# tashoyan/locations-recommender

Hardware: AMD Instinct MI355X
Metric: KNN person-pair cosines/s (cosine place+category, combine, top-K) (higher is better)
Workload: dtype u16 dot (exact, packed) / f64 cosine

## Files before the change

### include/locrec.h

```cpp
#ifndef LOCREC_H
#define LOCREC_H

#include <stdint.h>

#ifdef __cplusplus
extern "C" {
#endif

#define LOCREC_OK 0
#define LOCREC_E_INVALID_ARG 1
#define LOCREC_E_NOT_FOUND 2
#define LOCREC_E_DEVICE 3
#define LOCREC_E_OOM 4
#define LOCREC_E_ARITHMETIC 5

#define LOCREC_MEM_HOST 0
#define LOCREC_MEM_DEVICE 1

const char *locrec_last_error(void);
const char *locrec_version(void);

int32_t locrec_device_count(int32_t *out_count);
int32_t locrec_set_device(int32_t ordinal);
int32_t locrec_device_allocations(int64_t *out_count);
// ... 29 lines not shown

int32_t locrec_knn_destroy(locrec_knn_index *index);

int32_t locrec_knn_info(const locrec_knn_index *index, int64_t *out_n,
                        int64_t *out_scan_bytes, int32_t *out_packed);

int32_t locrec_knn_batch_scan_bytes(const locrec_knn_index *index, int64_t *out_scan_bytes);

int32_t locrec_knn_ht_image_info(const locrec_knn_index *index, int64_t *out_head_words, int64_t *out_tail_postings,
                                 int64_t *out_wide_rows);

int32_t locrec_knn_ht_multiplied_words(const locrec_knn_index *index, int64_t *out_words);

int32_t locrec_knn_ht_slice_counts(const locrec_knn_index *index, int64_t capacity, int32_t *out_place, int32_t *out_category,
                                   int64_t *out_slices);

int32_t locrec_knn_ht_last_hits(locrec_knn_index *index, int64_t nq, int64_t tile_capacity, int64_t off_capacity,
                                int64_t hit_capacity, int32_t *out_query_tile, int64_t *out_tiles, int32_t *out_slice0,
                                int32_t *out_nslices, int64_t *out_tile_base, uint32_t *out_off, uint32_t *out_hits,
                                int64_t *out_total);

int32_t locrec_knn_scan_plan(const locrec_knn_index *index, int32_t *out_kernel, int32_t *out_mode,
                             int32_t *out_query_tile, int32_t *out_waves_per_block);

int32_t locrec_knn_vector_lengths(locrec_knn_index *index, double *out_place_lengths,
                                  double *out_category_lengths);

int32_t locrec_knn_cosine_similarity(locrec_knn_index *index, int64_t person_a, int64_t person_b,
                                     double *out_place_cosine, double *out_category_cosine);

// ... 369 lines not shown
```

### locations-recommender_amd/_lib.py

```python
import ctypes as C
import os

import numpy as np

_HERE = os.path.dirname(os.path.abspath(__file__))
LIB_PATH = os.environ.get("LOCREC_LIB_PATH") or os.path.join(_HERE, "liblocrec.so")

OK, E_INVALID_ARG, E_NOT_FOUND, E_DEVICE, E_OOM, E_ARITHMETIC = 0, 1, 2, 3, 4, 5
MEM_HOST, MEM_DEVICE = 0, 1
KNN_BATCH_MAX_K = 1024
RANK_BATCH_MAX_N = 256


class IllegalArgumentException(ValueError):
    """What the reference throws for a failed require() or an unknown id
    (KnnRecommender.scala:17-20,83; StochasticRecommender.scala:33-34,70)."""


class LocrecRuntimeError(RuntimeError):
    """Device / allocation failures (the JNI shim maps these to RuntimeException)."""


_i64p = C.POINTER(C.c_int64)
_i32p = C.POINTER(C.c_int32)
# ... 13 lines not shown
    "locrec_cache_clear": [],
    "locrec_cache_stats": [_i64p, _i64p, _i64p, _i64p, _i64p],
    "locrec_knn_create": [C.c_int64, _i64p, _i64p, _i32p, _f64p, C.c_int32, _i64p, _i32p, _f64p, C.c_int32,
                          _i64p, _i64p, _i64p, C.POINTER(C.c_void_p)],
    "locrec_knn_create_from_device": [C.c_int64, C.c_void_p, C.c_void_p, C.c_void_p, C.c_void_p, C.c_int32, C.c_void_p, C.c_void_p,
                                      C.c_void_p, C.c_int32, C.c_void_p, C.c_void_p, C.c_void_p, C.POINTER(C.c_void_p)],
    "locrec_knn_destroy": [C.c_void_p],
    "locrec_knn_info": [C.c_void_p, _i64p, _i64p, _i32p],
    "locrec_knn_vector_lengths": [C.c_void_p, _f64p, _f64p],
    "locrec_knn_cosine_similarity": [C.c_void_p, C.c_int64, C.c_int64, _f64p, _f64p],
    "locrec_knn_scan_plan": [C.c_void_p, _i32p, _i32p, _i32p, _i32p],
    "locrec_knn_batch_scan_bytes": [C.c_void_p, _i64p],
    "locrec_knn_ht_image_info": [C.c_void_p, _i64p, _i64p, _i64p],
    "locrec_knn_ht_multiplied_words": [C.c_void_p, _i64p],
    "locrec_knn_ht_slice_counts": [C.c_void_p, C.c_int64, _i32p, _i32p, _i64p],
    "locrec_knn_ht_last_hits": [C.c_void_p, C.c_int64, C.c_int64, C.c_int64, C.c_int64, _i32p, _i64p, _i32p, _i32p, _i64p,
                                C.POINTER(C.c_uint32), C.POINTER(C.c_uint32), _i64p],
    "locrec_knn_query": [C.c_void_p, C.c_int64, C.c_double, C.c_double, C.c_int64, _i64p, _f64p, _i64p],
    "locrec_knn_recommend": [C.c_void_p, C.c_int64, C.c_double, C.c_double, C.c_int64, _i64p, _f64p, _i64p],
    "locrec_knn_recommend_batch": [C.c_void_p, C.c_int64, _i64p, C.c_double, C.c_double, C.c_int64,
                                   _i64p, _i64p, _f64p, _i64p],
    "locrec_knn_recommend_range_async": [C.c_void_p, C.c_int64, C.c_int64, C.c_double, C.c_double, C.c_int64],
    "locrec_knn_fetch_recommend": [C.c_void_p, C.c_int64, _i64p, _i64p, _f64p, _i64p],
    "locrec_knn_recommend_ranked_batch": [C.c_void_p, C.c_int64, _i64p, C.c_double, C.c_double, C.c_int64,
                                          C.c_int64, _i64p, _i64p, _i64p, C.c_int64, _i64p, _f64p, _i64p],
    "locrec_knn_fetch_ranked": [C.c_void_p, C.c_int64, C.c_int64, _i64p, _i64p, _i64p, C.c_int64, _i64p, _f64p, _i64p],
    "locrec_knn_recommend_ranked_batch_unvisited": [C.c_void_p, C.c_int64, _i64p, C.c_double, C.c_double, C.c_int64,
                                                    C.c_int64, _i64p, _i64p, _i64p, C.c_int64, _i64p, _f64p, _i64p],
    "locrec_knn_fetch_ranked_unvisited": [C.c_void_p, C.c_int64, C.c_int64, _i64p, _i64p, _i64p, C.c_int64, _i64p, _f64p, _i64p],
    "locrec_knn_query_shard": [C.c_void_p, C.c_int64, C.c_double, C.c_double, C.c_int64, C.c_int32, C.c_int32,
# ... 210 lines not shown
```

### locations-recommender_amd/csrc/knn.hip

```cpp

#include <algorithm>
#include <chrono>
#include <cstring>
#include <cmath>
#include <cstdlib>
#include <memory>
#include <new>
#include <numeric>
#include <type_traits>
#include <unordered_map>

#include "knn_index.h"

namespace {

using namespace locrec;

constexpr uint32_t kEmpty = 0xFFFFFFFFu;
constexpr int kMergeCap = 8192;
constexpr int kAggCap = 4096;
constexpr int kDirectMaxBytes = cfg::kDirectMaxBytes;
constexpr int kLdsSoftLimit = 64 * 1024;
constexpr int kLdsHardLimit = 160 * 1024;

struct Family {
    const uint32_t *sell;
// ... 1296 lines not shown
    ix->no_direct8 = std::getenv("LOCREC_KNN_NO_DIRECT8") != nullptr;
    ix->no_pack = std::getenv("LOCREC_KNN_NO_PACK") != nullptr;
    ix->no_seed = std::getenv("LOCREC_KNN_NO_SEED") != nullptr;
    ix->ht_round4 = std::getenv("LOCREC_KNN_HT_ROUND4") != nullptr;
    ix->no_tile_special = std::getenv("LOCREC_KNN_NO_TILE_SPECIAL") != nullptr;
    if (const char *e = std::getenv("LOCREC_KNN_SEED_MIN_SLICES")) ix->seed_min_slices = std::max(1, std::atoi(e));
    if (const char *e = std::getenv("LOCREC_KNN_SEED_SAMPLE")) ix->seed_sample_slices = std::max(8, std::atoi(e));
    ix->force_dense_query = std::getenv("LOCREC_KNN_FORCE_DENSE_QUERY") != nullptr;
    ix->ht.v1 = std::getenv("LOCREC_KNN_HT_V1") != nullptr;
    if (const char *e = std::getenv("LOCREC_KNN_HT_W")) {
        const int w = std::atoi(e);
        if (w == 6 || w == 8 || w == 12) ix->ht.waves = w;
    }
    if (ix->ht.v1) ix->ht.waves = 8;
    ix->ht.pre_v1 = std::getenv("LOCREC_KNN_HT_PRE_V1") != nullptr;
    if (const char *e = std::getenv("LOCREC_KNN_HT_PRE_STAGE"))
        ix->ht.pre_stage = std::min(kHtPreStageMax, std::max(kHtPreStageMin, std::atoi(e)));
    ix->force_generic = std::getenv("LOCREC_KNN_FORCE_GENERIC") != nullptr;
    ix->no_pack16 = std::getenv("LOCREC_KNN_NO_PACK16") != nullptr;
    ix->no_pop = std::getenv("LOCREC_KNN_NO_POP") != nullptr;
    ix->no_row_fallback = std::getenv("LOCREC_KNN_NO_ROW_FALLBACK") != nullptr;
    if (const char *e = std::getenv("LOCREC_KNN_HT_H")) ix->env_ht_h = std::max(4, std::atoi(e));
    if (const char *e = std::getenv("LOCREC_KNN_POP_H")) ix->env_pop_h = std::max(64, std::atoi(e));
    if (const char *e = std::getenv("LOCREC_KNN_BLOCKS")) ix->env_blocks = std::max(1, std::atoi(e));
    if (const char *e = std::getenv("LOCREC_KNN_FLUSH")) {
        const int v = std::atoi(e);
        if (v >= 1 && v <= 64 && (v & (v - 1)) == 0) ix->env_flush = v;
    }
    if (const char *e = std::getenv("LOCREC_KNN_ENTER")) ix->env_enter = std::max(0, std::atoi(e));
}
// ... 111 lines not shown
extern "C" int32_t locrec_knn_ht_slice_counts(const locrec_knn_index *ix, int64_t capacity, int32_t *out_place, int32_t *out_category,
                                              int64_t *out_slices) try
{
    if (!ix || !out_slices || capacity < 0 || (capacity > 0 && (!out_place || !out_category)))
        return fail(LOCREC_E_INVALID_ARG, "NULL argument");
    const bool have = ix->ht.ready && !ix->no_ht;
    const int64_t ns = have ? (int64_t)ix->ht.slice_cnt.size() : 0;
    *out_slices = ns;
    for (int64_t sl = 0; sl < std::min(ns, capacity); ++sl) {
        out_place[sl] = (int32_t)(ix->ht.slice_cnt[(size_t)sl] & 0xFFFFu);
        out_category[sl] = (int32_t)(ix->ht.slice_cnt[(size_t)sl] >> 16);
    }
    return LOCREC_OK;
} LOCREC_CATCH_ALL

extern "C" int32_t locrec_knn_scan_plan(const locrec_knn_index *ix, int32_t *out_kernel, int32_t *out_mode,
                                        int32_t *out_query_tile, int32_t *out_waves_per_block) try
{
    if (!ix) return fail(LOCREC_E_INVALID_ARG, "index is NULL");
    if (out_kernel) *out_kernel = ix->last_plan_kernel;
    if (out_mode) *out_mode = ix->last_plan_mode;
    if (out_query_tile) *out_query_tile = ix->last_plan_qt;
    if (out_waves_per_block) *out_waves_per_block = ix->last_plan_waves;
    return LOCREC_OK;
} LOCREC_CATCH_ALL

extern "C" int32_t locrec_knn_vector_lengths(locrec_knn_index *ix, double *out_p, double *out_c) try
{
    if (!ix) return fail(LOCREC_E_INVALID_ARG, "index is NULL");
    LOCREC_HIP_TRY(hipSetDevice(ix->device));
// ... 260 lines not shown
    std::vector<int64_t> ids((size_t)keff);
    std::vector<double> sims((size_t)keff);
    int64_t cnt = 0;
    LOCREC_TRY(locrec_knn_fetch_topk(ix, 1, keff, ids.data(), sims.data(), &cnt));
    const int64_t cap = *inout_count;
    for (int64_t i = 0; i < std::min(cap, cnt); ++i) {
        if (out_ids) out_ids[i] = ids[i];
        if (out_sims) out_sims[i] = sims[i];
    }
    *inout_count = cnt;
    return LOCREC_OK;
} LOCREC_CATCH_ALL

namespace {

int32_t enqueue_aggregate(locrec_knn_index *ix, int64_t nq, int K)
{
    hipStream_t s = ix->stream;
    const int64_t tmax = std::min<int64_t>((int64_t)K * std::max<int64_t>(1, ix->max_r_nnz), kAggCap);
    const int M = pow2ceil((int)std::max<int64_t>(2, tmax));
    LOCREC_TRY(ix->agg_place.reserve((size_t)nq * M));
    LOCREC_TRY(ix->agg_est.reserve((size_t)nq * M));
    LOCREC_TRY(ix->agg_n.reserve((size_t)nq));
    LOCREC_TRY(ix->agg_overflow.reserve((size_t)nq));
    const int M1 = std::min(M, 2048);
    const int threads1 = (M1 < M && K <= 512) ? 512 : kAggThreads;
    const int64_t nplaces = (int64_t)ix->cplace_ids.size();
    auto key32 = [&](int cap) { return ceil_log2i(nplaces + 2) + ceil_log2i(cap) <= 32; };
    auto lds_of = [&](int cap) { return (size_t)cap * (key32(cap) ? 14 : 18) + 8 + (size_t)K * 16 + (size_t)(K + 1) * 4 + 16; };
    const size_t lds_full = lds_of(M);
    auto launch = [&](int cap, int threads, int redo) -> int32_t {
        const size_t lds = lds_of(cap);
        if (key32(cap)) {
            if (lds > 64 * 1024)
                LOCREC_HIP_TRY(hipFuncSetAttribute(reinterpret_cast<const void *>(knn_aggregate<uint32_t>),
                                                   hipFuncAttributeMaxDynamicSharedMemorySize, (int)lds));
            hipLaunchKernelGGL(knn_aggregate<uint32_t>, dim3((unsigned)nq), dim3(threads), lds, s, ix->out_rows.p, ix->out_sims.p,
                               ix->out_cnt.p, K, ix->r_ptr.p, ix->r_pidx.p, ix->r_rating.p, ix->cplace_dev.p, cap,
                               ix->agg_place.p, ix->agg_est.p, ix->agg_n.p, ix->agg_overflow.p, (int64_t)M, redo, ceil_log2i(cap));
        } else {
            if (lds > 64 * 1024)
                LOCREC_HIP_TRY(hipFuncSetAttribute(reinterpret_cast<const void *>(knn_aggregate<uint64_t>),
                                                   hipFuncAttributeMaxDynamicSharedMemorySize, (int)lds));
            hipLaunchKernelGGL(knn_aggregate<uint64_t>, dim3((unsigned)nq), dim3(threads), lds, s, ix->out_rows.p, ix->out_sims.p,
                               ix->out_cnt.p, K, ix->r_ptr.p, ix->r_pidx.p, ix->r_rating.p, ix->cplace_dev.p, cap,
                               ix->agg_place.p, ix->agg_est.p, ix->agg_n.p, ix->agg_overflow.p, (int64_t)M, redo, 16);
        }
        return LOCREC_OK;
    };
    (void)lds_full;
    LOCREC_TRY(launch(M1, threads1, 0));
    if (M1 < M) LOCREC_TRY(launch(M, kAggThreads, 1));
    LOCREC_HIP_TRY(hipGetLastError());
    ix->agg_M = M;
    ix->have_agg = true;
    return LOCREC_OK;
}

int32_t enqueue_large_k_batch(locrec_knn_index *ix, const std::vector<int32_t> &rows, double pw, double cw, int64_t k)
{
    const int64_t nq = (int64_t)rows.size();
    ix->agg_rows = rows;
    ix->agg_first = -1;
    ix->agg_pw = pw;
    ix->agg_cw = cw;
    ix->last_nq = nq;
    ix->last_k = k;
    ix->single_pending = false;
// ... 282 lines not shown
            return fail(LOCREC_E_INVALID_ARG, "neighbour %lld is listed twice", (long long)ix->ids_row[*dup]);
    }
    LOCREC_HIP_TRY(hipSetDevice(ix->device));
    hipStream_t s = ix->stream;
    ix->have_result = false;
    ix->single_pending = false;
    if (n_neighbours <= LOCREC_KNN_BATCH_MAX_K) {
        const int K = (int)n_neighbours;
        const int64_t cnt = n_neighbours;
        LOCREC_TRY(ix->out_rows.reserve((size_t)K));
        LOCREC_TRY(ix->out_sims.reserve((size_t)K));
        LOCREC_TRY(ix->out_cnt.reserve(1));
        LOCREC_HIP_TRY(hipMemcpyAsync(ix->out_rows.p, rows.data(), (size_t)K * 4, hipMemcpyHostToDevice, s));
        LOCREC_HIP_TRY(hipMemcpyAsync(ix->out_sims.p, similarities, (size_t)K * 8, hipMemcpyHostToDevice, s));
        LOCREC_HIP_TRY(hipMemcpyAsync(ix->out_cnt.p, &cnt, 8, hipMemcpyHostToDevice, s));
        const int64_t tmax = std::min<int64_t>((int64_t)K * std::max<int64_t>(1, ix->max_r_nnz), kAggCap);
        const int M = pow2ceil((int)std::max<int64_t>(2, tmax));
        LOCREC_TRY(ix->agg_place.reserve((size_t)M));
        LOCREC_TRY(ix->agg_est.reserve((size_t)M));
        LOCREC_TRY(ix->agg_n.reserve(1));
        LOCREC_TRY(ix->agg_overflow.reserve(1));
        const size_t lds = (size_t)M * 18 + 8 + (size_t)K * 16 + (size_t)(K + 1) * 4 + 16;
        if (lds > 64 * 1024)
            LOCREC_HIP_TRY(hipFuncSetAttribute(reinterpret_cast<const void *>(knn_aggregate<uint64_t>),
                                               hipFuncAttributeMaxDynamicSharedMemorySize, (int)lds));
        hipLaunchKernelGGL(knn_aggregate<uint64_t>, dim3(1), dim3(kAggThreads), lds, s, ix->out_rows.p, ix->out_sims.p,
                           ix->out_cnt.p, K, ix->r_ptr.p, ix->r_pidx.p, ix->r_rating.p, ix->cplace_dev.p, M,
                           ix->agg_place.p, ix->agg_est.p, ix->agg_n.p, ix->agg_overflow.p, (int64_t)M, 0, 16);
        LOCREC_HIP_TRY(hipGetLastError());
        int64_t nout = 0;
        int32_t overflow = 0;
        std::vector<int64_t> hp((size_t)M);
        std::vector<double> he((size_t)M);
        LOCREC_HIP_TRY(hipMemcpyAsync(&nout, ix->agg_n.p, 8, hipMemcpyDeviceToHost, s));
        LOCREC_HIP_TRY(hipMemcpyAsync(&overflow, ix->agg_overflow.p, 4, hipMemcpyDeviceToHost, s));
        LOCREC_HIP_TRY(hipMemcpyAsync(hp.data(), ix->agg_place.p, (size_t)M * 8, hipMemcpyDeviceToHost, s));
        LOCREC_HIP_TRY(hipMemcpyAsync(he.data(), ix->agg_est.p, (size_t)M * 8, hipMemcpyDeviceToHost, s));
        LOCREC_HIP_TRY(hipStreamSynchronize(s));
        if (!overflow) {
            const int64_t w = std::min(*inout_count, nout);
            if (w > 0 && out_places) std::copy(hp.begin(), hp.begin() + w, out_places);
            if (w > 0 && out_ratings) std::copy(he.begin(), he.begin() + w, out_ratings);
            *inout_count = nout;
            return LOCREC_OK;
// ... 11 lines not shown
    if (!ix) return fail(LOCREC_E_INVALID_ARG, "index is NULL");
    if (!inout_count) return fail(LOCREC_E_INVALID_ARG, "inout_count is NULL");
    LOCREC_TRY(check_params(pw, cw, k));
    int32_t row = 0;
    LOCREC_TRY(find_query_row(ix, person_id, &row));
    const int64_t keff = std::min<int64_t>(k, std::max<int64_t>(1, ix->n - 1));
    LOCREC_HIP_TRY(hipSetDevice(ix->device));
    if (keff > LOCREC_KNN_BATCH_MAX_K)
        return knn_large_recommend(ix, row, pw, cw, keff, out_places, out_ratings, inout_count);
    hipStream_t s = ix->stream;
    static const bool dbg_timing = debug_env("LOCREC_DEBUG_TIMING") != nullptr;
    const auto tp0 = std::chrono::steady_clock::now();
    LOCREC_TRY(enqueue_topk(ix, nullptr, row, 1, ix->fp.nnz[row], ix->fc.nnz[row], pw, cw, keff));
    const auto tp1 = std::chrono::steady_clock::now();
    const int K = (int)keff;
    const int64_t tmax = std::min<int64_t>((int64_t)K * std::max<int64_t>(1, ix->max_r_nnz), kAggCap);
    const int M = pow2ceil((int)std::max<int64_t>(2, tmax));
    LOCREC_TRY(ix->agg_place.reserve((size_t)M));
    LOCREC_TRY(ix->agg_est.reserve((size_t)M));
    LOCREC_TRY(ix->agg_n.reserve(1));
    LOCREC_TRY(ix->agg_overflow.reserve(1));
    const size_t lds = (size_t)M * 18 + 8 + (size_t)K * 16 + (size_t)(K + 1) * 4 + 16;
    if (lds > 64 * 1024)
        LOCREC_HIP_TRY(hipFuncSetAttribute(reinterpret_cast<const void *>(knn_aggregate<uint64_t>),
                                           hipFuncAttributeMaxDynamicSharedMemorySize, (int)lds));
    unsigned char *agg_host = nullptr;
    if (ix->single_pending && !ix->last_scan_fast && (size_t)M * 16 + 64 <= locrec_knn_index::kStageBytes && stage_of(ix) &&
        ix->h_stage_dev && !ix->no_pack)
        agg_host = ix->h_stage_dev;
    hipLaunchKernelGGL(knn_aggregate<uint64_t>, dim3(1), dim3(kAggThreads), lds, s, ix->out_rows.p, ix->out_sims.p,
                       ix->out_cnt.p, K, ix->r_ptr.p, ix->r_pidx.p, ix->r_rating.p, ix->cplace_dev.p, M,
                       ix->agg_place.p, ix->agg_est.p, ix->agg_n.p, ix->agg_overflow.p, (int64_t)M, 0, 16, agg_host,
                       ix->sel1.p + 4, M);
    LOCREC_HIP_TRY(hipGetLastError());
    const auto tp2 = std::chrono::steady_clock::now();
    int64_t nout = 0;
    int32_t overflow = 0, overflow1 = 0, qoverflow = 0;
    std::vector<int64_t> hp_v;
    std::vector<double> he_v;
    const int64_t *hp = nullptr;
    const double *he = nullptr;
    unsigned char *st = (size_t)M * 16 + 64 <= locrec_knn_index::kStageBytes ? stage_of(ix) : nullptr;
    int64_t *p_nout = &nout;
    int32_t *p_flags = nullptr;
    int32_t local_flags[3] = {0, 0, 0};
    if (st) {
        p_nout = reinterpret_cast<int64_t *>(st);
        p_flags = reinterpret_cast<int32_t *>(st + 16);
        hp = reinterpret_cast<const int64_t *>(st + 64);
// ... 69 lines not shown
```

### locations-recommender_amd/csrc/knn_aggregate.h

```cpp
#pragma once

__device__ __forceinline__ int block_exclusive_scan(int v, int *wtot, int *total)
{
    const int lane = threadIdx.x & 63, wave = threadIdx.x >> 6, nw = blockDim.x >> 6;
    int inc = v;
#pragma unroll
    for (int d = 1; d < 64; d <<= 1) {
        const int o = __shfl_up(inc, d);
        if (lane >= d) inc += o;
    }
    if (lane == 63) wtot[wave] = inc;
    __syncthreads();
    if (threadIdx.x == 0) {
        int acc = 0;
        for (int w = 0; w < nw; ++w) {
            const int t = wtot[w];
            wtot[w] = acc;
            acc += t;
        }
        wtot[16] = acc;
    }
    __syncthreads();
    *total = wtot[16];
    return wtot[wave] + inc - v;
}

constexpr int kAggThreads = 1024;

template <typename KeyT>
__global__ __launch_bounds__(kAggThreads) void knn_aggregate(
    const int32_t *nb_rows, const double *nb_sims, const int64_t *nb_cnt, int32_t K,
    const int64_t *r_ptr, const int32_t *r_pidx, const double *r_rating, const int64_t *cplace_ids,
    int32_t M , int64_t *out_place, double *out_est, int64_t *out_n,
    int32_t *out_overflow, int64_t out_stride, int32_t redo_only, int32_t fbits,
    unsigned char *host = nullptr , const int32_t *host_flag_src = nullptr, int32_t host_cap = 0)
{
    if (redo_only && out_overflow[blockIdx.x] == 0) return;
    if (host && threadIdx.x == 0 && host_flag_src) *reinterpret_cast<int32_t *>(host + 20) = *host_flag_src;
    extern __shared__ __align__(16) unsigned char smem[];
    KeyT *key = reinterpret_cast<KeyT *>(smem);
    double *wrv = reinterpret_cast<double *>(smem + (((size_t)M * sizeof(KeyT) + 7) & ~(size_t)7));
    unsigned short *av = reinterpret_cast<unsigned short *>(wrv + M);
    int64_t *rbase = reinterpret_cast<int64_t *>(reinterpret_cast<unsigned char *>(av) + (((size_t)M * 2 + 7) & ~(size_t)7));
    double *simv = reinterpret_cast<double *>(rbase + K);
    int32_t *off = reinterpret_cast<int32_t *>(simv + K);
    const int q = blockIdx.x;
    const int tid = threadIdx.x;
    const int m = max(0, (int)nb_cnt[q]);
    const int32_t *rows = nb_rows + (int64_t)q * K;
    const double *sims = nb_sims + (int64_t)q * K;
// ... 7 lines not shown
    }
    int Tsum = 0;
    const int myoff = block_exclusive_scan(mycnt, wtot, &Tsum);
    if (tid < m) off[tid] = myoff;
    if (tid == 0) off[m] = Tsum;
    __syncthreads();
    const int T = min(Tsum, M + 1);
    if (T > M) {
        if (tid == 0) {
            out_overflow[q] = 1;
            out_n[q] = 0;
            if (host) {
                *reinterpret_cast<int32_t *>(host + 16) = 1;
                *reinterpret_cast<int64_t *>(host) = 0;
            }
        }
        return;
    }
    int n2 = 2;
    while (n2 < T) n2 <<= 1;
    auto neighbour_of = [&](int f) {
        int a = 0, b = m;
        while (b - a > 1) {
            const int mid = (a + b) >> 1;
            if (off[mid] <= f) a = mid; else b = mid;
        }
        return a;
    };
    for (int f = tid; f < n2; f += blockDim.x) {
        KeyT k = ~(KeyT)0;
        if (f < T) {
            const int a = neighbour_of(f);
            const int64_t e = rbase[a] + (f - off[a]);
// ... 68 lines not shown
                ss = ss + simv[av[f]];
            }
            const int64_t place = cplace_ids[pk];
            const double est = ws / ss;
            out_place[(int64_t)q * out_stride + o] = place;
            out_est[(int64_t)q * out_stride + o] = est;
            if (host) {
                h_place[o] = place;
                h_est[o] = est;
            }
            ++o;
        }
    }
}

__global__ __launch_bounds__(256) void knn_agg_compact(const int64_t *place, const double *est, const int64_t *out_n,
                                                       const int64_t *off, int64_t stride, int64_t *dense_place,
                                                       double *dense_est)
{
    const int q = blockIdx.x;
    const int64_t n = out_n[q], o = off[q];
    for (int64_t i = threadIdx.x; i < n; i += blockDim.x) {
        dense_place[o + i] = place[(int64_t)q * stride + i];
        dense_est[o + i] = est[(int64_t)q * stride + i];
    }
}

__global__ void knn_mark_absent(const double *norm_p, const double *norm_c, const int32_t *qrows, int32_t qrow0,
                                int32_t nq, int32_t K, int64_t *out_ids, double *out_sims, int32_t *out_rows,
                                int64_t *out_cnt)
// ... 13 lines not shown
```

### locations-recommender_amd/csrc/knn_index.h

```cpp
#pragma once

#include <algorithm>

#include "common.h"

namespace locrec {

namespace cfg {
constexpr int kDirectMaxBytes = 16384;
constexpr int kPopTable = 4096;
constexpr int kHtQt = 16;
constexpr int kHtHead = 512;
__host__ __device__ constexpr int ht_plane_rows(int h) { return h > kHtHead ? h : kHtHead; }
constexpr int kHtCatRows = 64;
constexpr int kHtNP = 4;
constexpr int kHtColdBytes = 512;
}

struct DevFamily {
    DevBuf<uint32_t> sell;
    DevBuf<double> sell_val;
    DevBuf<int64_t> sell_off;
    DevBuf<int32_t> sell_w;
    DevBuf<double> norm;
// ... 167 lines not shown
        int32_t qrow0;
        int64_t nq;
        int max_p, max_c;
        double pw, cw;
        int64_t k;
        bool mark_absent;
    } last_tiled{};
    bool single_pending = false;
    int32_t single_qrow = 0;
    double single_pw = 0, single_cw = 0;
    DevBuf<int64_t> agg_place, agg_n;
    DevBuf<double> agg_est;
    DevBuf<int32_t> agg_overflow;
    DevBuf<int64_t> agg_off, agg_dense_place;
    DevBuf<double> agg_dense_est;
    int agg_M = 0;
    bool have_agg = false;
    int32_t agg_first = 0;
    std::vector<int32_t> agg_rows;
    double agg_pw = 0, agg_cw = 0;
    KernelProfile prof;
    int last_plan_kernel = 0, last_plan_mode = 0, last_plan_qt = 0, last_plan_waves = 0;
    int64_t last_nq = 0, last_k = 0;
    bool have_result = false;
};

namespace locrec {

void knn_read_env(locrec_knn_index *ix);

// ... 20 lines not shown
```

### locations-recommender_amd/knn.py

```python
import ctypes as C

import numpy as np

from . import _cache
from . import _lib as L


class SparseVector:

    __slots__ = ("size", "indices", "values")

    def __init__(self, size, indices, values):
        self.size = int(size)
        self.indices = np.asarray(indices, dtype=np.int32)
        self.values = np.asarray(values, dtype=np.float64)
        if self.indices.shape != self.values.shape:
            raise L.IllegalArgumentException("requirement failed: Sparse vectors require that the dimension of the "
                                             "indices match the dimension of the values.")


def _vectors_to_csr(person_ids, frame):
    by_id = {int(p): v for p, v in zip(frame["person_id"], frame["rating_vector"])}
    sizes = {v.size for v in by_id.values()}
    if len(sizes) > 1:
# ... 98 lines not shown
        return {"head_words": v[0].value, "tail_postings": v[1].value, "wide_rows": v[2].value}

    def ht_multiplied_words(self):
        v = C.c_int64()
        L.check(L.lib().locrec_knn_ht_multiplied_words(self._h, C.byref(v)))
        return v.value

    def ht_slice_counts(self):
        ns = C.c_int64()
        L.check(L.lib().locrec_knn_ht_slice_counts(self._h, 0, None, None, C.byref(ns)))
        p, c = np.zeros(ns.value, np.int32), np.zeros(ns.value, np.int32)
        if ns.value:
            L.check(L.lib().locrec_knn_ht_slice_counts(self._h, ns.value, p.ctypes.data_as(C.POINTER(C.c_int32)),
                                                       c.ctypes.data_as(C.POINTER(C.c_int32)), C.byref(ns)))
        return np.stack([p, c], axis=1)

    def ht_last_hits(self, nq):
        qt, s0, s1 = C.c_int32(), C.c_int32(), C.c_int32()
        nt, total = C.c_int64(), C.c_int64()
        u32p = C.POINTER(C.c_uint32)
        head = [C.byref(x) for x in (qt, nt, s0, s1)]
        L.check(L.lib().locrec_knn_ht_last_hits(self._h, int(nq), 0, 0, 0, *head, None, None, None, C.byref(total)))
        base = np.zeros(nt.value + 1, np.int64)
        off = np.zeros((nt.value, s1.value - s0.value + 1), np.uint32)
        hits = np.zeros(total.value, np.uint32)
        L.check(L.lib().locrec_knn_ht_last_hits(self._h, int(nq), base.size, off.size, hits.size, *head, L.ptr(base, C.c_int64),
                                                off.ctypes.data_as(u32p), hits.ctypes.data_as(u32p), C.byref(total)))
        return {"query_tile": qt.value, "tiles": nt.value, "slice0": s0.value, "nslices": s1.value, "tile_base": base,
                "off": off, "hits": hits}

# ... 325 lines not shown
```

Before: 1029 billion.

## Add bitmap-bucket aggregation kernel as default first pass before sort fallback

Adds a new aggregation kernel that groups neighbour ratings by place through an LDS bitmap, popcount prefix ranks and per-slot buckets, replacing the key sort in the first pass. A planner picks the bucket form when LDS and capacity allow, and falls back to the existing sort kernel as a redo pass for overflowing or heavy-bucket queries. It also adds device-side stats counters updated by atomics. This targets the recommendation aggregation stage, not the cosine/top-K scan the metric counts, so its effect on the metric is probably small.

Result: faster. 1061 billion (median of 6 runs) (+3.1%).

```diff
diff --git a/include/locrec.h b/include/locrec.h
--- a/include/locrec.h
+++ b/include/locrec.h
@@ -67,6 +67,8 @@
 
 int32_t locrec_knn_ht_slice_counts(const locrec_knn_index *index, int64_t capacity, int32_t *out_place, int32_t *out_category,
                                    int64_t *out_slices);
+
+int32_t locrec_knn_aggregate_stats(locrec_knn_index *index, int64_t out[3]);
 
 int32_t locrec_knn_ht_last_hits(locrec_knn_index *index, int64_t nq, int64_t tile_capacity, int64_t off_capacity,
                                 int64_t hit_capacity, int32_t *out_query_tile, int64_t *out_tiles, int32_t *out_slice0,
diff --git a/locations-recommender_amd/_lib.py b/locations-recommender_amd/_lib.py
--- a/locations-recommender_amd/_lib.py
+++ b/locations-recommender_amd/_lib.py
@@ -51,6 +51,7 @@
     "locrec_knn_ht_image_info": [C.c_void_p, _i64p, _i64p, _i64p],
     "locrec_knn_ht_multiplied_words": [C.c_void_p, _i64p],
     "locrec_knn_ht_slice_counts": [C.c_void_p, C.c_int64, _i32p, _i32p, _i64p],
+    "locrec_knn_aggregate_stats": [C.c_void_p, _i64p],
     "locrec_knn_ht_last_hits": [C.c_void_p, C.c_int64, C.c_int64, C.c_int64, C.c_int64, _i32p, _i64p, _i32p, _i32p, _i64p,
                                 C.POINTER(C.c_uint32), C.POINTER(C.c_uint32), _i64p],
     "locrec_knn_query": [C.c_void_p, C.c_int64, C.c_double, C.c_double, C.c_int64, _i64p, _f64p, _i64p],
diff --git a/locations-recommender_amd/csrc/knn.hip b/locations-recommender_amd/csrc/knn.hip
--- a/locations-recommender_amd/csrc/knn.hip
+++ b/locations-recommender_amd/csrc/knn.hip
@@ -10,6 +10,7 @@
 #include <type_traits>
 #include <unordered_map>
 
+#include "knn_agg_plan.h"
 #include "knn_index.h"
 
 namespace {
@@ -1336,6 +1337,7 @@
     }
     if (ix->ht.v1) ix->ht.waves = 8;
     ix->ht.pre_v1 = std::getenv("LOCREC_KNN_HT_PRE_V1") != nullptr;
+    ix->agg_sort = std::getenv("LOCREC_KNN_AGG_SORT") != nullptr;
     if (const char *e = std::getenv("LOCREC_KNN_HT_PRE_STAGE"))
         ix->ht.pre_stage = std::min(kHtPreStageMax, std::max(kHtPreStageMin, std::atoi(e)));
     ix->force_generic = std::getenv("LOCREC_KNN_FORCE_GENERIC") != nullptr;
@@ -1477,6 +1479,20 @@
     return LOCREC_OK;
 } LOCREC_CATCH_ALL
 
+extern "C" int32_t locrec_knn_aggregate_stats(locrec_knn_index *ix, int64_t out[3]) try
+{
+    if (!ix || !out) return fail(LOCREC_E_INVALID_ARG, "NULL argument");
+    out[0] = out[1] = out[2] = 0;
+    if (!ix->agg_stats.p) return LOCREC_OK;
+    LOCREC_HIP_TRY(hipSetDevice(ix->device));
+    unsigned long long h[3] = {0, 0, 0};
+    LOCREC_HIP_TRY(hipMemcpyAsync(h, ix->agg_stats.p, sizeof h, hipMemcpyDeviceToHost, ix->stream));
+    LOCREC_HIP_TRY(hipMemsetAsync(ix->agg_stats.p, 0, sizeof h, ix->stream));
+    LOCREC_HIP_TRY(hipStreamSynchronize(ix->stream));
+    for (int i = 0; i < 3; ++i) out[i] = (int64_t)h[i];
+    return LOCREC_OK;
+} LOCREC_CATCH_ALL
+
 extern "C" int32_t locrec_knn_scan_plan(const locrec_knn_index *ix, int32_t *out_kernel, int32_t *out_mode,
                                         int32_t *out_query_tile, int32_t *out_waves_per_block) try
 {
@@ -1767,44 +1783,61 @@
 
 namespace {
 
+KnnAggPlan aggregate_plan(const locrec_knn_index *ix, int K)
+{
+    return knn_agg_plan(K, ix->max_r_nnz, (int64_t)ix->cplace_ids.size(), kAggCap, ix->agg_sort);
+}
+
+int32_t launch_aggregate(locrec_knn_index *ix, const KnnAggLaunch &l, int64_t nq, int K, int M, int redo, bool last,
+                         unsigned char *host = nullptr, const int32_t *host_flag_src = nullptr, int32_t host_cap = 0)
+{
+    hipStream_t s = ix->stream;
+    if (!ix->agg_stats.p) {
+        LOCREC_TRY(ix->agg_stats.alloc(3));
+        LOCREC_HIP_TRY(hipMemsetAsync(ix->agg_stats.p, 0, 3 * sizeof(unsigned long long), s));
+    }
+    const void *fn = l.form == kAggBuckets ? reinterpret_cast<const void *>(knn_aggregate_buckets)
+                     : l.key32             ? reinterpret_cast<const void *>(knn_aggregate<uint32_t>)
+                                           : reinterpret_cast<const void *>(knn_aggregate<uint64_t>);
+    if (l.lds > 64 * 1024)
+        LOCREC_HIP_TRY(hipFuncSetAttribute(fn, hipFuncAttributeMaxDynamicSharedMemorySize, (int)l.lds));
+    const dim3 grid((unsigned)nq), block((unsigned)l.threads);
+    if (l.form == kAggBuckets)
+        hipLaunchKernelGGL(knn_aggregate_buckets, grid, block, l.lds, s, ix->out_rows.p, ix->out_sims.p, ix->out_cnt.p, K,
+                           ix->r_ptr.p, ix->r_pidx.p, ix->r_rating.p, ix->cplace_dev.p, l.cap, (int32_t)ix->cplace_ids.size(),
+                           kAggBucketMax, ix->agg_place.p, ix->agg_est.p, ix->agg_n.p, ix->agg_overflow.p, (int64_t)M, host,
+                           host_flag_src, host_cap, ix->agg_stats.p, (int32_t)last);
+    else if (l.key32)
+        hipLaunchKernelGGL(knn_aggregate<uint32_t>, grid, block, l.lds, s, ix->out_rows.p, ix->out_sims.p, ix->out_cnt.p, K,
+                           ix->r_ptr.p, ix->r_pidx.p, ix->r_rating.p, ix->cplace_dev.p, l.cap, ix->agg_place.p, ix->agg_est.p,
+                           ix->agg_n.p, ix->agg_overflow.p, (int64_t)M, redo, l.fbits, host, host_flag_src, host_cap,
+                           ix->agg_stats.p, (int32_t)last);
+    else
+        hipLaunchKernelGGL(knn_aggregate<uint64_t>, grid, block, l.lds, s, ix->out_rows.p, ix->out_sims.p, ix->out_cnt.p, K,
+                           ix->r_ptr.p, ix->r_pidx.p, ix->r_rating.p, ix->cplace_dev.p, l.cap, ix->agg_place.p, ix->agg_est.p,
+                           ix->agg_n.p, ix->agg_overflow.p, (int64_t)M, redo, l.fbits, host, host_flag_src, host_cap,
+                           ix->agg_stats.p, (int32_t)last);
+    return LOCREC_OK;
+}
+
+int32_t launch_aggregate_plan(locrec_knn_index *ix, const KnnAggPlan &plan, int64_t nq, int K, unsigned char *host = nullptr,
+                              const int32_t *host_flag_src = nullptr, int32_t host_cap = 0)
+{
+    LOCREC_TRY(launch_aggregate(ix, plan.pass1, nq, K, plan.M, 0, !plan.redo_needed, host, host_flag_src, host_cap));
+    if (plan.redo_needed) LOCREC_TRY(launch_aggregate(ix, plan.redo, nq, K, plan.M, 1, true, host, host_flag_src, host_cap));
+    LOCREC_HIP_TRY(hipGetLastError());
+    return LOCREC_OK;
+}
+
 int32_t enqueue_aggregate(locrec_knn_index *ix, int64_t nq, int K)
 {
-    hipStream_t s = ix->stream;
-    const int64_t tmax = std::min<int64_t>((int64_t)K * std::max<int64_t>(1, ix->max_r_nnz), kAggCap);
-    const int M = pow2ceil((int)std::max<int64_t>(2, tmax));
+    const KnnAggPlan plan = aggregate_plan(ix, K);
+    const int M = plan.M;
     LOCREC_TRY(ix->agg_place.reserve((size_t)nq * M));
     LOCREC_TRY(ix->agg_est.reserve((size_t)nq * M));
     LOCREC_TRY(ix->agg_n.reserve((size_t)nq));
     LOCREC_TRY(ix->agg_overflow.reserve((size_t)nq));
-    const int M1 = std::min(M, 2048);
-    const int threads1 = (M1 < M && K <= 512) ? 512 : kAggThreads;
-    const int64_t nplaces = (int64_t)ix->cplace_ids.size();
-    auto key32 = [&](int cap) { return ceil_log2i(nplaces + 2) + ceil_log2i(cap) <= 32; };
-    auto lds_of = [&](int cap) { return (size_t)cap * (key32(cap) ? 14 : 18) + 8 + (size_t)K * 16 + (size_t)(K + 1) * 4 + 16; };
-    const size_t lds_full = lds_of(M);
-    auto launch = [&](int cap, int threads, int redo) -> int32_t {
-        const size_t lds = lds_of(cap);
-        if (key32(cap)) {
-            if (lds > 64 * 1024)
-                LOCREC_HIP_TRY(hipFuncSetAttribute(reinterpret_cast<const void *>(knn_aggregate<uint32_t>),
-                                                   hipFuncAttributeMaxDynamicSharedMemorySize, (int)lds));
-            hipLaunchKernelGGL(knn_aggregate<uint32_t>, dim3((unsigned)nq), dim3(threads), lds, s, ix->out_rows.p, ix->out_sims.p,
-                               ix->out_cnt.p, K, ix->r_ptr.p, ix->r_pidx.p, ix->r_rating.p, ix->cplace_dev.p, cap,
-                               ix->agg_place.p, ix->agg_est.p, ix->agg_n.p, ix->agg_overflow.p, (int64_t)M, redo, ceil_log2i(cap));
-        } else {
-            if (lds > 64 * 1024)
-                LOCREC_HIP_TRY(hipFuncSetAttribute(reinterpret_cast<const void *>(knn_aggregate<uint64_t>),
-                                                   hipFuncAttributeMaxDynamicSharedMemorySize, (int)lds));
-            hipLaunchKernelGGL(knn_aggregate<uint64_t>, dim3((unsigned)nq), dim3(threads), lds, s, ix->out_rows.p, ix->out_sims.p,
-                               ix->out_cnt.p, K, ix->r_ptr.p, ix->r_pidx.p, ix->r_rating.p, ix->cplace_dev.p, cap,
-                               ix->agg_place.p, ix->agg_est.p, ix->agg_n.p, ix->agg_overflow.p, (int64_t)M, redo, 16);
-        }
-        return LOCREC_OK;
-    };
-    (void)lds_full;
-    LOCREC_TRY(launch(M1, threads1, 0));
-    if (M1 < M) LOCREC_TRY(launch(M, kAggThreads, 1));
-    LOCREC_HIP_TRY(hipGetLastError());
+    LOCREC_TRY(launch_aggregate_plan(ix, plan, nq, K));
     ix->agg_M = M;
     ix->have_agg = true;
     return LOCREC_OK;
@@ -2117,20 +2150,13 @@
         LOCREC_HIP_TRY(hipMemcpyAsync(ix->out_rows.p, rows.data(), (size_t)K * 4, hipMemcpyHostToDevice, s));
         LOCREC_HIP_TRY(hipMemcpyAsync(ix->out_sims.p, similarities, (size_t)K * 8, hipMemcpyHostToDevice, s));
         LOCREC_HIP_TRY(hipMemcpyAsync(ix->out_cnt.p, &cnt, 8, hipMemcpyHostToDevice, s));
-        const int64_t tmax = std::min<int64_t>((int64_t)K * std::max<int64_t>(1, ix->max_r_nnz), kAggCap);
-        const int M = pow2ceil((int)std::max<int64_t>(2, tmax));
+        const KnnAggPlan plan = aggregate_plan(ix, K);
+        const int M = plan.M;
         LOCREC_TRY(ix->agg_place.reserve((size_t)M));
         LOCREC_TRY(ix->agg_est.reserve((size_t)M));
         LOCREC_TRY(ix->agg_n.reserve(1));
         LOCREC_TRY(ix->agg_overflow.reserve(1));
-        const size_t lds = (size_t)M * 18 + 8 + (size_t)K * 16 + (size_t)(K + 1) * 4 + 16;
-        if (lds > 64 * 1024)
-            LOCREC_HIP_TRY(hipFuncSetAttribute(reinterpret_cast<const void *>(knn_aggregate<uint64_t>),
-                                               hipFuncAttributeMaxDynamicSharedMemorySize, (int)lds));
-        hipLaunchKernelGGL(knn_aggregate<uint64_t>, dim3(1), dim3(kAggThreads), lds, s, ix->out_rows.p, ix->out_sims.p,
-                           ix->out_cnt.p, K, ix->r_ptr.p, ix->r_pidx.p, ix->r_rating.p, ix->cplace_dev.p, M,
-                           ix->agg_place.p, ix->agg_est.p, ix->agg_n.p, ix->agg_overflow.p, (int64_t)M, 0, 16);
-        LOCREC_HIP_TRY(hipGetLastError());
+        LOCREC_TRY(launch_aggregate_plan(ix, plan, 1, K));
         int64_t nout = 0;
         int32_t overflow = 0;
         std::vector<int64_t> hp((size_t)M);
@@ -2172,25 +2198,17 @@
     LOCREC_TRY(enqueue_topk(ix, nullptr, row, 1, ix->fp.nnz[row], ix->fc.nnz[row], pw, cw, keff));
     const auto tp1 = std::chrono::steady_clock::now();
     const int K = (int)keff;
-    const int64_t tmax = std::min<int64_t>((int64_t)K * std::max<int64_t>(1, ix->max_r_nnz), kAggCap);
-    const int M = pow2ceil((int)std::max<int64_t>(2, tmax));
+    const KnnAggPlan plan = aggregate_plan(ix, K);
+    const int M = plan.M;
     LOCREC_TRY(ix->agg_place.reserve((size_t)M));
     LOCREC_TRY(ix->agg_est.reserve((size_t)M));
     LOCREC_TRY(ix->agg_n.reserve(1));
     LOCREC_TRY(ix->agg_overflow.reserve(1));
-    const size_t lds = (size_t)M * 18 + 8 + (size_t)K * 16 + (size_t)(K + 1) * 4 + 16;
-    if (lds > 64 * 1024)
-        LOCREC_HIP_TRY(hipFuncSetAttribute(reinterpret_cast<const void *>(knn_aggregate<uint64_t>),
-                                           hipFuncAttributeMaxDynamicSharedMemorySize, (int)lds));
     unsigned char *agg_host = nullptr;
     if (ix->single_pending && !ix->last_scan_fast && (size_t)M * 16 + 64 <= locrec_knn_index::kStageBytes && stage_of(ix) &&
         ix->h_stage_dev && !ix->no_pack)
         agg_host = ix->h_stage_dev;
-    hipLaunchKernelGGL(knn_aggregate<uint64_t>, dim3(1), dim3(kAggThreads), lds, s, ix->out_rows.p, ix->out_sims.p,
-                       ix->out_cnt.p, K, ix->r_ptr.p, ix->r_pidx.p, ix->r_rating.p, ix->cplace_dev.p, M,
-                       ix->agg_place.p, ix->agg_est.p, ix->agg_n.p, ix->agg_overflow.p, (int64_t)M, 0, 16, agg_host,
-                       ix->sel1.p + 4, M);
-    LOCREC_HIP_TRY(hipGetLastError());
+    LOCREC_TRY(launch_aggregate_plan(ix, plan, 1, K, agg_host, ix->sel1.p + 4, M));
     const auto tp2 = std::chrono::steady_clock::now();
     int64_t nout = 0;
     int32_t overflow = 0, overflow1 = 0, qoverflow = 0;
diff --git a/locations-recommender_amd/csrc/knn_agg_plan.h b/locations-recommender_amd/csrc/knn_agg_plan.h
--- /dev/null
+++ b/locations-recommender_amd/csrc/knn_agg_plan.h
@@ -0,0 +1,141 @@
+#pragma once
+
+#include <algorithm>
+#include <cstddef>
+#include <cstdint>
+
+#if defined(__HIPCC__)
+#define LOCREC_AGG_HD __host__ __device__
+#else
+#define LOCREC_AGG_HD
+#endif
+
+namespace locrec {
+
+constexpr int kAggThreads = 1024;
+constexpr int kAggPass1Cap = 2048;
+constexpr int kAggPer = 4;
+constexpr int kAggBucketMax = 128;
+constexpr size_t kAggLdsMax = 160 * 1024;
+constexpr size_t kAggBucketLdsMax = 80 * 1024;
+
+LOCREC_AGG_HD inline int32_t knn_agg_words(int64_t nplaces) { return (int32_t)((nplaces + 31) >> 5); }
+LOCREC_AGG_HD inline int32_t knn_agg_word_of(uint32_t p) { return (int32_t)(p >> 5); }
+LOCREC_AGG_HD inline uint32_t knn_agg_bit_of(uint32_t p) { return 1u << (p & 31); }
+LOCREC_AGG_HD inline int32_t knn_agg_rank_in_word(uint32_t word, uint32_t p)
+{
+    return __builtin_popcount(word & (knn_agg_bit_of(p) - 1u));
+}
+LOCREC_AGG_HD inline int32_t knn_agg_slot(int32_t prefix, uint32_t word, uint32_t p) { return prefix + knn_agg_rank_in_word(word, p); }
+LOCREC_AGG_HD inline int32_t knn_agg_words_per_thread(int32_t words, int32_t threads) { return (words + threads - 1) / threads; }
+
+LOCREC_AGG_HD inline size_t knn_agg_up8(size_t b) { return (b + 7) & ~(size_t)7; }
+LOCREC_AGG_HD inline size_t knn_agg_lds_neighbours(int K) { return (size_t)K * 16 + (size_t)(K + 1) * 4; }
+LOCREC_AGG_HD inline size_t knn_agg_lds_sort(int cap, int K, bool key32)
+{
+    return (size_t)cap * (key32 ? 14 : 18) + 8 + knn_agg_lds_neighbours(K) + 16;
+}
+struct KnnAggBucketLds {
+    size_t bitmap, prefix, prod, nb, start, place, entry, neighbours, total;
+};
+LOCREC_AGG_HD inline KnnAggBucketLds knn_agg_bucket_lds(int cap, int K, int64_t nplaces)
+{
+    const size_t words = (size_t)knn_agg_words(nplaces);
+    KnnAggBucketLds l{};
+    l.bitmap = 0;
+    l.prefix = l.bitmap + knn_agg_up8(words * 4);
+    const size_t ranked = l.prefix + knn_agg_up8(words * 2);
+    l.prod = 0;
+    l.nb = l.prod + (size_t)cap * 8;
+    const size_t ordered = l.nb + knn_agg_up8((size_t)cap * 2);
+    l.start = ranked > ordered ? ranked : ordered;
+    l.place = l.start + knn_agg_up8((size_t)(cap + 1) * 4);
+    l.entry = l.place + knn_agg_up8((size_t)cap * 4);
+    l.neighbours = l.entry + knn_agg_up8((size_t)cap * 2);
+    l.total = l.neighbours + knn_agg_up8(knn_agg_lds_neighbours(K));
+    return l;
+}
+
+inline int knn_agg_pow2ceil(int64_t v)
+{
+    int p = 1;
+    while (p < v) p <<= 1;
+    return p;
+}
+inline int knn_agg_ceil_log2(int64_t v)
+{
+    int b = 0;
+    while (((int64_t)1 << b) < v) ++b;
+    return b;
+}
+
+enum KnnAggForm : int32_t { kAggNone = 0, kAggBuckets = 1, kAggSort = 2 };
+
+struct KnnAggLaunch {
+    int32_t form = kAggNone;
+    int32_t cap = 0;
+    int32_t threads = 0;
+    size_t lds = 0;
+    bool key32 = false;
+    int32_t fbits = 16;
+};
+
+struct KnnAggPlan {
+    int32_t M = 0;
+    KnnAggLaunch pass1, redo;
+    bool redo_needed = false;
+};
+
+inline KnnAggLaunch knn_agg_sort_launch(int cap, int threads, int K, int64_t nplaces)
+{
+    KnnAggLaunch l;
+    l.form = kAggSort;
+    l.cap = cap;
+    l.threads = threads;
+    l.key32 = knn_agg_ceil_log2(nplaces + 2) + knn_agg_ceil_log2(cap) <= 32;
+    l.fbits = l.key32 ? knn_agg_ceil_log2(cap) : 16;
+    l.lds = knn_agg_lds_sort(cap, K, l.key32);
+    return l;
+}
+
+inline int knn_agg_pass1_threads(int K, int cap1, int M) { return (cap1 < M && K <= 512) ? 512 : kAggThreads; }
+
+inline KnnAggPlan knn_agg_plan(int K, int64_t max_r_nnz, int64_t nplaces, int agg_cap, bool force_sort,
+                               int bucket_max = kAggBucketMax)
+{
+    KnnAggPlan p;
+    const int64_t rows_max = (int64_t)K * std::max<int64_t>(1, max_r_nnz);
+    const int64_t tmax = std::min<int64_t>(rows_max, agg_cap);
+    p.M = knn_agg_pow2ceil(std::max<int64_t>(2, tmax));
+    const int cap1 = std::min(p.M, kAggPass1Cap);
+    const int threads1 = knn_agg_pass1_threads(K, cap1, p.M);
+    const size_t blds = knn_agg_bucket_lds(cap1, K, nplaces).total;
+    const bool buckets = !force_sort && blds <= kAggBucketLdsMax && cap1 <= threads1 * kAggPer;
+    if (buckets) {
+        p.pass1.form = kAggBuckets;
+        p.pass1.cap = cap1;
+        p.pass1.threads = threads1;
+        p.pass1.lds = blds;
+    } else {
+        p.pass1 = knn_agg_sort_launch(cap1, threads1, K, nplaces);
+    }
+    const bool rows_flag = rows_max > cap1 && cap1 < p.M;
+    const bool bucket_flag = buckets && rows_max > bucket_max;
+    p.redo_needed = rows_flag || bucket_flag;
+    if (p.redo_needed) p.redo = knn_agg_sort_launch(p.M, kAggThreads, K, nplaces);
+    return p;
+}
+
+inline int64_t knn_agg_place_limit(int K, int64_t max_r_nnz, int agg_cap)
+{
+    int64_t lo = 0, hi = (int64_t)1 << 32;
+    if (knn_agg_plan(K, max_r_nnz, 1, agg_cap, false).pass1.form != kAggBuckets) return 0;
+    lo = 1;
+    while (hi - lo > 1) {
+        const int64_t mid = lo + (hi - lo) / 2;
+        if (knn_agg_plan(K, max_r_nnz, mid, agg_cap, false).pass1.form == kAggBuckets) lo = mid; else hi = mid;
+    }
+    return lo;
+}
+
+}
diff --git a/locations-recommender_amd/csrc/knn_aggregate.h b/locations-recommender_amd/csrc/knn_aggregate.h
--- a/locations-recommender_amd/csrc/knn_aggregate.h
+++ b/locations-recommender_amd/csrc/knn_aggregate.h
@@ -25,7 +25,6 @@
     return wtot[wave] + inc - v;
 }
 
-constexpr int kAggThreads = 1024;
 
 template <typename KeyT>
 __global__ __launch_bounds__(kAggThreads) void knn_aggregate(
@@ -33,7 +32,9 @@
     const int64_t *r_ptr, const int32_t *r_pidx, const double *r_rating, const int64_t *cplace_ids,
     int32_t M , int64_t *out_place, double *out_est, int64_t *out_n,
     int32_t *out_overflow, int64_t out_stride, int32_t redo_only, int32_t fbits,
-    unsigned char *host = nullptr , const int32_t *host_flag_src = nullptr, int32_t host_cap = 0)
+    unsigned char *host = nullptr , const int32_t *host_flag_src = nullptr, int32_t host_cap = 0,
+    unsigned long long *stats = nullptr ,
+    int32_t last_pass = 1 )
 {
     if (redo_only && out_overflow[blockIdx.x] == 0) return;
     if (host && threadIdx.x == 0 && host_flag_src) *reinterpret_cast<int32_t *>(host + 20) = *host_flag_src;
@@ -71,9 +72,11 @@
                 *reinterpret_cast<int32_t *>(host + 16) = 1;
                 *reinterpret_cast<int64_t *>(host) = 0;
             }
+            if (stats && last_pass) atomicAdd(&stats[2], 1ull);
         }
         return;
     }
+    if (stats && tid == 0) atomicAdd(&stats[1], 1ull);
     int n2 = 2;
     while (n2 < T) n2 <<= 1;
     auto neighbour_of = [&](int f) {
@@ -172,6 +175,185 @@
     }
 }
 
+__global__ __launch_bounds__(kAggThreads) void knn_aggregate_buckets(
+    const int32_t *nb_rows, const double *nb_sims, const int64_t *nb_cnt, int32_t K,
+    const int64_t *r_ptr, const int32_t *r_pidx, const double *r_rating, const int64_t *cplace_ids,
+    int32_t M , int32_t nplaces, int32_t bucket_max, int64_t *out_place, double *out_est,
+    int64_t *out_n, int32_t *out_overflow, int64_t out_stride, unsigned char *host, const int32_t *host_flag_src,
+    int32_t host_cap, unsigned long long *stats, int32_t last_pass)
+{
+    if (host && threadIdx.x == 0 && host_flag_src) *reinterpret_cast<int32_t *>(host + 20) = *host_flag_src;
+    extern __shared__ __align__(16) unsigned char smem[];
+    const KnnAggBucketLds L = knn_agg_bucket_lds(M, K, nplaces);
+    double *sprod = reinterpret_cast<double *>(smem + L.prod);
+    int32_t *start = reinterpret_cast<int32_t *>(smem + L.start);
+    int32_t *splace = reinterpret_cast<int32_t *>(smem + L.place);
+    unsigned short *entry = reinterpret_cast<unsigned short *>(smem + L.entry);
+    unsigned short *snb = reinterpret_cast<unsigned short *>(smem + L.nb);
+    uint32_t *bitmap = reinterpret_cast<uint32_t *>(smem + L.bitmap);
+    unsigned short *prefix = reinterpret_cast<unsigned short *>(smem + L.prefix);
+    int64_t *rbase = reinterpret_cast<int64_t *>(smem + L.neighbours);
+    double *simv = reinterpret_cast<double *>(rbase + K);
+    int32_t *off = reinterpret_cast<int32_t *>(simv + K);
+    const int q = blockIdx.x;
+    const int tid = threadIdx.x, nthreads = (int)blockDim.x;
+    const int m = max(0, (int)nb_cnt[q]);
+    const int32_t *rows = nb_rows + (int64_t)q * K;
+    const double *sims = nb_sims + (int64_t)q * K;
+    const int cap = min(M, nthreads * kAggPer);
+    const int nwords = knn_agg_words(nplaces);
+    __shared__ int wtot[17];
+    for (int w = tid; w < nwords; w += nthreads) bitmap[w] = 0u;
+    int mycnt = 0;
+    if (tid < m) {
+        const int64_t b = r_ptr[rows[tid]];
+        rbase[tid] = b;
+        simv[tid] = sims[tid];
+        mycnt = (int32_t)min(r_ptr[rows[tid] + 1] - b, (int64_t)cap + 1);
+    }
+    int Tsum = 0;
+    const int myoff = block_exclusive_scan(mycnt, wtot, &Tsum);
+    if (tid < m) off[tid] = myoff;
+    if (tid == 0) off[m] = Tsum;
+    __syncthreads();
+    auto flag_query = [&]() {
+        if (tid == 0) {
+            out_overflow[q] = 1;
+            out_n[q] = 0;
+            if (host) {
+                *reinterpret_cast<int32_t *>(host + 16) = 1;
+                *reinterpret_cast<int64_t *>(host) = 0;
+            }
+            if (stats && last_pass) atomicAdd(&stats[2], 1ull);
+        }
+    };
+    const int T = min(Tsum, cap + 1);
+    if (T > cap) {
+        flag_query();
+        return;
+    }
+    auto neighbour_of = [&](int f) {
+        int a = 0, b = m;
+        while (b - a > 1) {
+            const int mid = (a + b) >> 1;
+            if (off[mid] <= f) a = mid; else b = mid;
+        }
+        return a;
+    };
+    int32_t pidx[kAggPer], nbr[kAggPer];
+    double prod[kAggPer];
+    int bad = 0;
+#pragma unroll
+    for (int j = 0; j < kAggPer; ++j) {
+        const int f = tid + j * nthreads;
+        pidx[j] = -1;
+        nbr[j] = 0;
+        prod[j] = 0.0;
+        if (f < T) {
+            const int a = neighbour_of(f);
+            const int64_t e = rbase[a] + (f - off[a]);
+            const int32_t p = r_pidx[e];
+            if ((uint32_t)p < (uint32_t)nplaces) {
+                pidx[j] = p;
+                nbr[j] = a;
+                prod[j] = r_rating[e] * simv[a];
+                atomicOr(&bitmap[knn_agg_word_of((uint32_t)p)], knn_agg_bit_of((uint32_t)p));
+            } else {
+                bad = 1;
+            }
+        }
+    }
+    __syncthreads();
+    const int wpt = knn_agg_words_per_thread(nwords, nthreads);
+    const int w0 = min(tid * wpt, nwords), w1 = min(w0 + wpt, nwords);
+    int pc = 0;
+    for (int w = w0; w < w1; ++w) pc += __popc(bitmap[w]);
+    int nslots = 0;
+    int run = block_exclusive_scan(pc, wtot, &nslots);
+    for (int w = w0; w < w1; ++w) {
+        prefix[w] = (unsigned short)run;
+        run += __popc(bitmap[w]);
+    }
+    for (int s = tid; s <= nslots; s += nthreads) start[s] = 0;
+    __syncthreads();
+    int32_t slot[kAggPer], arrival[kAggPer];
+#pragma unroll
+    for (int j = 0; j < kAggPer; ++j) {
+        slot[j] = 0;
+        arrival[j] = 0;
+        if (pidx[j] >= 0) {
+            const int w = knn_agg_word_of((uint32_t)pidx[j]);
+            slot[j] = knn_agg_slot(prefix[w], bitmap[w], (uint32_t)pidx[j]);
+            arrival[j] = atomicAdd(&start[slot[j]], 1);
+        }
+    }
+    __syncthreads();
+    const int per = max(1, (cap + nthreads - 1) / nthreads);
+    const int lo = min(tid * per, nslots), hi = min(lo + per, nslots);
+    int mine = 0;
+    for (int s = lo; s < hi; ++s) {
+        const int c = start[s];
+        mine += c;
+        bad |= c > bucket_max;
+    }
+    int total = 0;
+    int first = block_exclusive_scan(mine, wtot, &total);
+    for (int s = lo; s < hi; ++s) {
+        const int c = start[s];
+        start[s] = first;
+        first += c;
+    }
+    if (tid == 0) start[nslots] = total;
+    if (__syncthreads_or(bad)) {
+        flag_query();
+        return;
+    }
+#pragma unroll
+    for (int j = 0; j < kAggPer; ++j)
+        if (pidx[j] >= 0) {
+            entry[start[slot[j]] + arrival[j]] = (unsigned short)(tid + j * nthreads);
+            splace[slot[j]] = pidx[j];
+        }
+    __syncthreads();
+#pragma unroll
+    for (int j = 0; j < kAggPer; ++j)
+        if (pidx[j] >= 0) {
+            const int f = tid + j * nthreads;
+            const int b = start[slot[j]], e = start[slot[j] + 1];
+            int r = b;
+            for (int i = b; i < e; ++i) r += (int)entry[i] < f;
+            sprod[r] = prod[j];
+            snb[r] = (unsigned short)nbr[j];
+        }
+    __syncthreads();
+    if (tid == 0) {
+        out_n[q] = nslots;
+        out_overflow[q] = 0;
+        if (host) {
+            *reinterpret_cast<int32_t *>(host + 16) = 0;
+            *reinterpret_cast<int64_t *>(host) = nslots;
+        }
+        if (stats) atomicAdd(&stats[0], 1ull);
+    }
+    int64_t *h_place = host ? reinterpret_cast<int64_t *>(host + 64) : nullptr;
+    double *h_est = host ? reinterpret_cast<double *>(host + 64 + (size_t)host_cap * 8) : nullptr;
+    for (int s = tid; s < nslots; s += nthreads) {
+        double ws = 0.0, ss = 0.0;
+        for (int t = start[s], e = start[s + 1]; t < e; ++t) {
+            ws = ws + sprod[t];
+            ss = ss + simv[snb[t]];
+        }
+        const int64_t place = cplace_ids[splace[s]];
+        const double est = ws / ss;
+        out_place[(int64_t)q * out_stride + s] = place;
+        out_est[(int64_t)q * out_stride + s] = est;
+        if (host) {
+            h_place[s] = place;
+            h_est[s] = est;
+        }
+    }
+}
+
 __global__ __launch_bounds__(256) void knn_agg_compact(const int64_t *place, const double *est, const int64_t *out_n,
                                                        const int64_t *off, int64_t stride, int64_t *dense_place,
                                                        double *dense_est)
diff --git a/locations-recommender_amd/csrc/knn_index.h b/locations-recommender_amd/csrc/knn_index.h
--- a/locations-recommender_amd/csrc/knn_index.h
+++ b/locations-recommender_amd/csrc/knn_index.h
@@ -205,6 +205,8 @@
     DevBuf<int32_t> agg_overflow;
     DevBuf<int64_t> agg_off, agg_dense_place;
     DevBuf<double> agg_dense_est;
+    bool agg_sort = false;
+    DevBuf<unsigned long long> agg_stats;
     int agg_M = 0;
     bool have_agg = false;
     int32_t agg_first = 0;
diff --git a/locations-recommender_amd/knn.py b/locations-recommender_amd/knn.py
--- a/locations-recommender_amd/knn.py
+++ b/locations-recommender_amd/knn.py
@@ -136,6 +136,11 @@
             L.check(L.lib().locrec_knn_ht_slice_counts(self._h, ns.value, p.ctypes.data_as(C.POINTER(C.c_int32)),
                                                        c.ctypes.data_as(C.POINTER(C.c_int32)), C.byref(ns)))
         return np.stack([p, c], axis=1)
+
+    def aggregate_stats(self):
+        v = (C.c_int64 * 3)()
+        L.check(L.lib().locrec_knn_aggregate_stats(self._h, v))
+        return {"buckets": int(v[0]), "sort": int(v[1]), "flagged": int(v[2])}
 
     def ht_last_hits(self, nq):
         qt, s0, s1 = C.c_int32(), C.c_int32(), C.c_int32()
```
